# mingyuanzhou/SiD-LSG

Measured on AMD Instinct MI355X. Metric: distillation images/sec (512^2, SD1.5, kappa=1.5), higher is better.
Workload: dtype bf16

## Files before the change

### include/sidlsg_hip.h

```cpp
#ifndef SIDLSG_HIP_H
#define SIDLSG_HIP_H
#ifdef __cplusplus
extern "C" {
#endif

#define SIDLSG_OUT_F32 1
#define SIDLSG_SILU 2
#define SIDLSG_ACCUM 4

int sidlsg_gemm_bf16(const void* A, int lda, const void* W, void* C, int ldc, const float* bias, const void* res, int ldres,
                     const float* rowvec, int ld_rowvec, int rows_per_batch, int M, int N, int K, float alpha, int flags,
                     void* stream);

int sidlsg_conv3x3_bf16(const void* X, int ldx, const void* W, void* Y, int ldc, const float* bias, const void* res, int ldres,
                        const float* rowvec, int ld_rowvec, int B, int H, int Wd, int Cin, int Cout, int stride, int ups,
                        float alpha, int flags, void* stream);

int sidlsg_gemm_geglu_ok(int M, int N2, int K);
int sidlsg_gemm_geglu_bf16(const void* A, int lda, const void* W, void* H, int ldh, void* Y, int ldy, const float* bias, int M, int N2,
                           int K, void* stream);

int sidlsg_gemm_geglu_bwd_ok(int M, int F, int K);
int sidlsg_gemm_geglu_bwd_bf16(const void* dOut, int lda, const void* Wt, const void* H, void* dH, int ldh, int M, int F, int K,
                               void* stream);
int sidlsg_gemm_geglu_bf16_g2(const void* A, int lda, const void* W, const void* W1, void* H, int ldh, void* Y, int ldy, const float* bias,
                              const float* bias1, int M, int N2, int K, void* stream);
int sidlsg_gemm_geglu_bwd_bf16_g2(const void* dOut, int lda, const void* Wt, const void* Wt1, const void* H, void* dH, int ldh, int M, int F,
                                  int K, void* stream);

int sidlsg_set_workspace(void* ptr, long long bytes);
int sidlsg_set_stream_workspace(void* stream, void* ptr, long long bytes);

int sidlsg_wgrad_bf16(const void* dY, int ldy, const void* A, int lda, float* dW, float* dBias, int M, int N, int K,
                      void* stream);
int sidlsg_wgrad_assign_bf16(const void* dY, int ldy, const void* A, int lda, float* dW, float* dBias, int M, int N, int K,
                             void* stream);
int sidlsg_wgrad_group_bf16(const void* jobs, int njobs, void* stream);
int sidlsg_wgrad_group160_bf16(const void* jobs, int njobs, void* stream);
int sidlsg_conv3x3_wgrad_assign_bf16(const void* dY, int ldy, const void* X, int ldx, float* dW, float* dBias, int B, int H, int Wd,
                                     int Cin, int Cout, int stride, int ups, void* stream);
int sidlsg_debug_wgrad_blocks_per_cu(int which);
int sidlsg_debug_set_p8(int mode);
int sidlsg_conv3x3_wgrad_bf16(const void* dY, int ldy, const void* X, int ldx, float* dW, float* dBias, int B, int H, int Wd,
                              int Cin, int Cout, int stride, int ups, void* stream);

int sidlsg_groupnorm_ws_floats(int B, int HW, int C, int G);
int sidlsg_groupnorm_nchunks(int B, int HW, int C, int G);
int sidlsg_groupnorm_fwd(const void* x, const float* gamma, const float* beta, void* y, float* stats, float* ws, int B,
                         int HW, int C, int G, float eps, int silu, void* stream);
int sidlsg_groupnorm_bwd(const void* x, const void* dy, const float* stats, const float* gamma, const float* beta,
                         const void* dres, void* dx, float* dgamma, float* dbeta, float* ws, int B, int HW, int C, int G,
                         int silu, void* stream);
int sidlsg_layernorm_fwd(const void* x, const float* gamma, const float* beta, void* y, float* stats, int rows, int C,
                         float eps, void* stream);
int sidlsg_layernorm_bwd_nblocks(int rows);
int sidlsg_defer_reductions(void* stream, int on);
int sidlsg_flush_reductions(void* stream);
int sidlsg_pending_reductions(void* stream);
int sidlsg_layernorm_bwd(const void* x, const void* dy, const float* stats, const float* gamma, const void* dres, void* dx,
                         float* dgamma, float* dbeta, float* ws, int rows, int C, void* stream);

int sidlsg_gemm_bf16_g2(const void* A, int lda, const void* W, const void* W1, void* C, int ldc, const float* bias, const float* bias1,
                        const void* res, int ldres, const float* rowvec, int ld_rowvec, int rows_per_batch, int M, int N, int K,
                        float alpha, int flags, void* stream);
int sidlsg_conv3x3_bf16_g2(const void* X, int ldx, const void* W, const void* W1, void* Y, int ldc, const float* bias, const float* bias1,
                           const void* res, int ldres, const float* rowvec, int ld_rowvec, int B, int H, int Wd, int Cin, int Cout,
                           int stride, int ups, float alpha, int flags, void* stream);
int sidlsg_groupnorm_fwd_g2(const void* x, const float* gamma, const float* beta, const float* gamma1, const float* beta1, void* y,
                            float* stats, float* ws, int B, int HW, int C, int G, float eps, int silu, void* stream);
int sidlsg_groupnorm_bwd_g2(const void* x, const void* dy, const float* stats, const float* gamma, const float* beta, const float* gamma1,
                            const float* beta1, const void* dres, void* dx, float* ws, int B, int HW, int C, int G, int silu,
                            void* stream);
int sidlsg_layernorm_fwd_g2(const void* x, const float* gamma, const float* beta, const float* gamma1, const float* beta1, void* y,
                            float* stats, int rows, int C, float eps, void* stream);
int sidlsg_layernorm_bwd_g2(const void* x, const void* dy, const float* stats, const float* gamma, const float* gamma1, const void* dres,
                            void* dx, int rows, int C, void* stream);

int sidlsg_trace_enable(int max_kernels);
int sidlsg_trace_pause(int paused);
int sidlsg_trace_set_stride(int family, int stride);
int sidlsg_trace_read(int family, double* out);

int sidlsg_attn_fwd(const void* Q, const void* K, const void* V, void* O, float* LSE, int B, int H, int Nq, int Nk, int D,
                    int ldq, int ldk, int ldv, int ldo, long long bsq, long long bsk, long long bsv, long long bso,
                    void* stream);
int sidlsg_attn_bwd(const void* Q, const void* K, const void* V, const void* O, const void* dO, const float* LSE, void* dQ,
                    void* dK, void* dV, float* delta, int B, int H, int Nq, int Nk, int D, int ldq, int ldk, int ldv, int ldo,
                    long long bsq, long long bsk, long long bsv, long long bso, void* stream);
int sidlsg_attn_fwd_ps(const void* Q, const void* K, const void* V, void* O, float* LSE, int B, int H, int Nq, int Nk, int D,
                       int ldq, int ldk, int ldv, int ldo, long long bsq, long long bsk, long long bsv, long long bso,
                       void* stream);
int sidlsg_attn_bwd_ps(const void* Q, const void* K, const void* V, const void* O, const void* dO, const float* LSE, void* dQ,
                       void* dK, void* dV, float* delta, int B, int H, int Nq, int Nk, int D, int ldq, int ldk, int ldv, int ldo,
                       long long bsq, long long bsk, long long bsv, long long bso, void* stream);

int sidlsg_noisy_input(const float* x0, const float* noise, const float* s0, const float* s1, void* out, float* xt, int B,
                       int C, int HW, int Cp, int dup, void* stream);
int sidlsg_noisy_input_bwd(const void* g, const float* s0, float* dx0, int B, int C, int HW, int Cp, int dup, int accumulate,
                           void* stream);
int sidlsg_cfg_x0(const float* eps, const float* xt, const float* s0, const float* s1, float* out, int B, int C, int HW,
                  int Ce, int dup, float kappa, int predict_x0, void* stream);
int sidlsg_cfg_x0_bwd(const float* g, const float* s0, const float* s1, void* deps, float* dxt, int B, int C, int HW, int Cp,
                      int dup, float kappa, int predict_x0, void* stream);

int sidlsg_g_loss(const float* x, const float* yr, const float* yf, float* dx, float* dyr, float* dyf, float* loss, float* ws,
                  int S, int n, float alpha, float scale, void* stream);
int sidlsg_fake_loss(const float* e, const float* noise, float* de, float* loss, float* ws, int S, int n, float scale,
                     void* stream);

int sidlsg_adam_ema(float* p, float* g, float* m, float* v, float* ema, void* w_bf16, const float* hyper, long long n,
                    int zero_grad, void* stream);

int sidlsg_timestep_embed(const long long* t, void* out, int B, int dim, void* stream);
int sidlsg_silu_fwd(const void* x, void* y, long long n, void* stream);
int sidlsg_silu_bwd(const void* x, const void* dy, void* dx, long long n, void* stream);
int sidlsg_geglu_fwd(const void* h, void* y, long long M, int F, void* stream);
int sidlsg_geglu_bwd(const void* h, const void* dy, void* dh, long long M, int F, void* stream);
int sidlsg_concat2(void* a, void* b, void* out, long long M, int C1, int C2, int to_parts, void* stream);
int sidlsg_sumpool2x2(const void* g, void* out, int B, int H, int W, int C, void* stream);
int sidlsg_zero_insert2(const void* g, void* out, int B, int Ho, int Wo, int H, int W, int C, void* stream);
int sidlsg_add_bf16(const void* a, const void* b, void* o, long long n, void* stream);
int sidlsg_colsum_nchunks(int B, int rows_per_batch);
int sidlsg_colsum(const void* g, int ldg, float* per_batch, float* total, float* ws, int B, int rows_per_batch, int N,
                  void* stream);
int sidlsg_colsum_strided(const void* g, int ldg, float* per_batch, int ld_pb, float* total, int B, int rows_per_batch, int N, void* stream);
int sidlsg_cast_f32_bf16(const float* x, void* y, long long n, void* stream);
int sidlsg_cast_bf16_f32(const void* x, float* y, long long n, void* stream);
int sidlsg_transpose_w(const float* src, void* dst, int N, int K, int T, void* stream);
int sidlsg_transpose_w_batched(const void* jobs, int njobs, int nblocks, void* stream);
int sidlsg_transpose_w16_batched(const void* jobs, int njobs, int nblocks, void* stream);
int sidlsg_scale_cast_ranges(const void* jobs, int njobs, int nblocks, void* stream);

int sidlsg_bias_act(const void* x, const void* b, const void* dy, void* out, long long n, int stepB, int sizeB, int act,
                    float alpha, float gain, float clamp, int grad, int dtype, void* stream);

int sidlsg_quantize_fp8_rows(const void* src_bf16, void* dst_fp8, float* scale, int rows, int cols, void* stream);
int sidlsg_gemm_fp8w(const void* A, int lda, const void* W8, const float* wscale, void* C, int ldc, const float* bias, const void* res,
                     int ldres, const float* rowvec, int ld_rowvec, int rows_per_batch, int M, int N, int K, float alpha,
                     int flags, void* stream);
int sidlsg_conv3x3_fp8w(const void* X, int ldx, const void* W8, const float* wscale, void* Y, int ldc, const float* bias,
                        const void* res, int ldres, const float* rowvec, int ld_rowvec, int B, int H, int Wd, int Cin, int Cout,
                        int stride, int ups, float alpha, int flags, void* stream);
int sidlsg_cast_fp8(const void* src_bf16, void* dst_fp8, long long n, void* stream);
int sidlsg_conv3x3_mx8(const void* X8, int ldx, const void* W8, const float* wscale, void* Y, int ldc, const float* bias, const void* res,
                       int ldres, const float* rowvec, int ld_rowvec, int B, int H, int Wd, int Cin, int Cout, float alpha, int flags,
                       void* stream);
int sidlsg_layernorm_fwd_fp8(const void* x, const float* gamma, const float* beta, void* y8, float* stats, int rows, int C,
                             float eps, void* stream);
int sidlsg_groupnorm_fwd_fp8(const void* x, const float* gamma, const float* beta, void* y8, float* stats, float* ws, int B,
                             int HW, int C, int G, float eps, int silu, void* stream);
int sidlsg_gemm_mx8(const void* A8, int lda, const void* W8, const float* wscale, void* C, int ldc, const float* bias, const void* res,
                    int ldres, const float* rowvec, int ld_rowvec, int rows_per_batch, int M, int N, int K, float alpha,
                    int flags, void* stream);

int sidlsg_gemm_f32(const void* A, int lda, const void* W, void* C, int ldc, const float* bias, const void* res, int ldres,
                    const float* rowvec, int ld_rowvec, int rows_per_batch, int M, int N, int K, float alpha, int flags,
                    void* stream);
int sidlsg_conv3x3_f32(const void* X, int ldx, const void* W, void* Y, int ldc, const float* bias, const void* res, int ldres,
                       const float* rowvec, int ld_rowvec, int B, int H, int Wd, int Cin, int Cout, int stride, int ups,
                       float alpha, int flags, void* stream);
int sidlsg_wgrad_f32(const void* dY, int ldy, const void* A, int lda, float* dW, float* dBias, int M, int N, int K,
                     void* stream);
int sidlsg_conv3x3_wgrad_f32(const void* dY, int ldy, const void* X, int ldx, float* dW, float* dBias, int B, int H, int Wd,
                             int Cin, int Cout, int stride, int ups, void* stream);
int sidlsg_groupnorm_fwd_f32(const void* x, const float* gamma, const float* beta, void* y, float* stats, float* ws, int B,
                             int HW, int C, int G, float eps, int silu, void* stream);
int sidlsg_groupnorm_bwd_f32(const void* x, const void* dy, const float* stats, const float* gamma, const float* beta,
                             const void* dres, void* dx, float* dgamma, float* dbeta, float* ws, int B, int HW, int C, int G,
                             int silu, void* stream);
int sidlsg_layernorm_fwd_f32(const void* x, const float* gamma, const float* beta, void* y, float* stats, int rows, int C,
                             float eps, void* stream);
int sidlsg_layernorm_bwd_f32(const void* x, const void* dy, const float* stats, const float* gamma, const void* dres, void* dx,
                             float* dgamma, float* dbeta, float* ws, int rows, int C, void* stream);
int sidlsg_attn_fwd_f32(const void* Q, const void* K, const void* V, void* O, float* LSE, int B, int H, int Nq, int Nk, int D,
                        int ldq, int ldk, int ldv, int ldo, long long bsq, long long bsk, long long bsv, long long bso,
                        void* stream);
int sidlsg_attn_bwd_f32(const void* Q, const void* K, const void* V, const void* O, const void* dO, const float* LSE, void* dQ,
// ... 28 lines not shown
```

### sid_lsg_amd/csrc/attention.hip

```cpp
#include "common.h"
#include <stdlib.h>
#include <type_traits>

struct AttnParams {
    const bf16 *Q, *K, *V, *dO;
    bf16 *O, *dQ, *dK, *dV;
    float* LSE;
    const float* delta;
    float* delta_out;
    int B, H, Nq, Nk, D;
    int ldq, ldk, ldv, ldo;
    long long bsq, bsk, bsv, bso;
    float scale2;
    float scale;
    int xcd;
    int rot;
};

DEVFN void attn_block_coords(const AttnParams& p, int& bx, int& h, int& b) {
    bx = blockIdx.x; h = blockIdx.y; b = blockIdx.z;
    if (!p.xcd) return;
    const unsigned nx = gridDim.x, ny = gridDim.y, total = nx * ny * gridDim.z;
    unsigned L = blockIdx.x + nx * (blockIdx.y + ny * blockIdx.z);
    const unsigned q = total >> 3, r = total & 7, xcd = L & 7, idx = L >> 3;
// ... 532 lines not shown
        const float* dl_c = dl_s[pb_] + sub * AK_QT;
        f32x4 pp[KT][4], ds[KT][4];
        ATTN_PRIO(8, 1);
#pragma unroll
        for (int qt = 0; qt < 4; qt++) {
            Frag<DP> fq, fdo;
            frag_from_lds<DP>(fq, Qs + (qt * 16 + li) * LD, lg);
            frag_from_lds<DP>(fdo, dOs + (qt * 16 + li) * LD, lg);
#pragma unroll
            for (int kt = 0; kt < KT; kt++) {
                if constexpr (PS) {
                    const f32x4 nl = *reinterpret_cast<const f32x4*>(&lse_c[qt * 16 + lg * 4]);
                    const f32x4 nd = *reinterpret_cast<const f32x4*>(&dl_c[qt * 16 + lg * 4]);
                    const f32x4 s = mma_d<DP>(nl, fq, fk[kt]);
                    const f32x4 dp = mma_d<DP>(nd, fdo, fv[kt]);
#pragma unroll
                    for (int r = 0; r < 4; r++) {
                        const float pr = __builtin_amdgcn_exp2f(s[r]);
                        pp[kt][qt][r] = pr;
                        ds[kt][qt][r] = pr * dp[r];
                    }
                } else {
                const f32x4 s = mma_d<DP>((f32x4){0, 0, 0, 0}, fq, fk[kt]);
                const f32x4 dp = mma_d<DP>((f32x4){0, 0, 0, 0}, fdo, fv[kt]);
#pragma unroll
                for (int r = 0; r < 4; r++) {
                    const int ql = qt * 16 + lg * 4 + r;
                    const float pr = __builtin_amdgcn_exp2f(fmaf(s[r], p.scale2, -lse_c[ql]));
                    pp[kt][qt][r] = pr;
                    ds[kt][qt][r] = pr * (dp[r] - dl_c[ql]);
                }
                }
            }
        }
        ATTN_PRIO(8, 0);
        ATTN_PRIO(4, 1);
#pragma unroll
        for (int half = 0; half < 2; half++)
#pragma unroll
            for (int dt = 0; dt < DT; dt++) {
                const bf16x8 fa = tr_frag32(dOs, LD, 32 * half, dt * 16, li, lg);
                const bf16x8 fb = tr_frag32(Qs, LD, 32 * half, dt * 16, li, lg);
#pragma unroll
                for (int kt = 0; kt < KT; kt++) {
                    const bf16x8 pbv = pack_p(pp[kt][2 * half], pp[kt][2 * half + 1]);
                    const bf16x8 dsb = pack_p(ds[kt][2 * half], ds[kt][2 * half + 1]);
                    dv[kt][dt] = __builtin_amdgcn_mfma_f32_16x16x32_bf16(fa, pbv, dv[kt][dt], 0, 0, 0);
                    dk[kt][dt] = __builtin_amdgcn_mfma_f32_16x16x32_bf16(fb, dsb, dk[kt][dt], 0, 0, 0);
                }
            }
        ATTN_PRIO(4, 0);
        }
        if (more) {
            pb_ ^= 1;
            tq.commit(Qs2[pb_], LD); tdo.commit(dOs2[pb_], LD);
            if (threadIdx.x < ST) { lse_s[pb_][threadIdx.x] = lse_r; dl_s[pb_][threadIdx.x] = dl_r; }
            __syncthreads();
        }
    };
    {
        int q0 = 0;
        for (; q0 < p.Nq; q0 += ST) qtile(q0, std::true_type{});
    }
#pragma unroll
    for (int kt = 0; kt < KT; kt++) {
        if (!kok[kt]) continue;
        const int key = key0 + kt * 16 + li;
        bf16* dKp = p.dK + b * p.bsk + (long long)key * p.ldk + (long long)h * p.D;
        bf16* dVp = p.dV + b * p.bsv + (long long)key * p.ldv + (long long)h * p.D;
#pragma unroll
        for (int dt = 0; dt < DT; dt++) {
            const int d = dt * 16 + lg * 4;
            if (d + 4 <= p.D) {
                const float kf = PS ? 0.6931471805599453f : p.scale;
                bf16x4 a = {f2bf(dk[kt][dt][0] * kf), f2bf(dk[kt][dt][1] * kf), f2bf(dk[kt][dt][2] * kf), f2bf(dk[kt][dt][3] * kf)};
                bf16x4 c = {f2bf(dv[kt][dt][0]), f2bf(dv[kt][dt][1]), f2bf(dv[kt][dt][2]), f2bf(dv[kt][dt][3])};
                *reinterpret_cast<bf16x4*>(dKp + d) = a;
                *reinterpret_cast<bf16x4*>(dVp + d) = c;
            }
        }
    }
}

#define ATTN_INST(DP, PS)                                                            \
    template __global__ void attn_q_kernel<DP, 2, 0, true, PS>(AttnParams);           \
    template __global__ void attn_q_kernel<DP, 2, 0, false, PS>(AttnParams);          \
    template __global__ void attn_q_kernel<DP, 2, 1, false, PS>(AttnParams);          \
    template __global__ void attn_dkdv_kernel<DP, 1, PS>(AttnParams);
#define ATTN_INST2(DP) ATTN_INST(DP, false) ATTN_INST(DP, true)
ATTN_INST2(16) ATTN_INST2(32) ATTN_INST2(48) ATTN_INST2(64) ATTN_INST2(80) ATTN_INST2(96) ATTN_INST2(128) ATTN_INST2(160)
template __global__ void attn_dkdv_kernel<48, 2, false>(AttnParams);
template __global__ void attn_dkdv_kernel<48, 2, true>(AttnParams);
#undef ATTN_INST
#undef ATTN_INST2

template <int DP, int QT, bool PS>
static int launch_attn_q(const AttnParams& p, int mode, hipStream_t s) {
    const int qb = 4 * QT * 16;
    if (mode == 0) {
        if (p.D == DP - 8) SIDLSG_LAUNCH((attn_q_kernel<DP, QT, 0, true, PS>), dim3((p.Nq + qb - 1) / qb, p.H, p.B), dim3(256), 0, s, p);
        else SIDLSG_LAUNCH((attn_q_kernel<DP, QT, 0, false, PS>), dim3((p.Nq + qb - 1) / qb, p.H, p.B), dim3(256), 0, s, p);
    } else SIDLSG_LAUNCH((attn_q_kernel<DP, QT, 1, false, PS>), dim3((p.Nq + qb - 1) / qb, p.H, p.B), dim3(256), 0, s, p);
    return sidlsg_last_error();
}
template <int DP, int KT, bool PS>
static int launch_attn_dkdv(const AttnParams& p, hipStream_t s) {
    const int kb = 4 * KT * 16;
    SIDLSG_LAUNCH((attn_dkdv_kernel<DP, KT, PS>), dim3((p.Nk + kb - 1) / kb, p.H, p.B), dim3(256), 0, s, p);
    return sidlsg_last_error();
}
template <int DP, int QT, int KT, bool PS>
static int launch_attn(const AttnParams& p, int mode, hipStream_t s) {
    return mode == 2 ? launch_attn_dkdv<DP, KT, PS>(p, s) : launch_attn_q<DP, QT, PS>(p, mode, s);
}
static int attn_xcd_on(int mode, const AttnParams& p) {
    static const int mask = getenv("SIDLSG_ATTN_XCD") ? atoi(getenv("SIDLSG_ATTN_XCD")) : 15;
    if (!((mask >> mode) & 1)) return 0;
    return mode == 0 || (mask & 8) || (p.Nq <= 1024 && p.Nk <= 1024);
}
static int attn_rot_on(int mode, const AttnParams& p) {
    static const int mask = getenv("SIDLSG_ATTN_ROT") ? atoi(getenv("SIDLSG_ATTN_ROT")) : 6;
    return p.xcd && ((mask >> mode) & 1);
}
template <bool PS>
static int dispatch_attn(const AttnParams& p_in, int mode, hipStream_t s) {
    AttnParams p = p_in;
    p.xcd = attn_xcd_on(mode, p);
    p.rot = attn_rot_on(mode, p);
    if (p.D % 8 || p.D <= 0 || p.D > 160) return SIDLSG_EINVAL;
    const int dp = (p.D + 15) / 16 * 16;
    static const bool allow_kt2 = !(getenv("SIDLSG_ATTN_KT2") && atoi(getenv("SIDLSG_ATTN_KT2")) == 0);
    const bool kt2 = allow_kt2 && mode == 2 && p.Nk >= 1024;
    switch (dp) {
        case 16: return launch_attn<16, 2, 1, PS>(p, mode, s);
        case 32: return launch_attn<32, 2, 1, PS>(p, mode, s);
        case 48: return kt2 ? launch_attn<48, 2, 2, PS>(p, mode, s) : launch_attn<48, 2, 1, PS>(p, mode, s);
        case 64: return launch_attn<64, 2, 1, PS>(p, mode, s);
        case 80: return launch_attn<80, 2, 1, PS>(p, mode, s);
        case 96: return launch_attn<96, 2, 1, PS>(p, mode, s);
        case 128: return launch_attn<128, 2, 1, PS>(p, mode, s);
        case 160: return launch_attn<160, 2, 1, PS>(p, mode, s);
    }
    return SIDLSG_EINVAL;
}

static bool attn_spans_ok(int Nq, int Nk, int ldq, int ldk, int ldv, int ldo) {
    const long long lim = 0x7FFFFFFFLL / 2;
    return (long long)Nq * ldq < lim && (long long)Nk * ldk < lim && (long long)Nk * ldv < lim && (long long)Nq * ldo < lim;
}
static int attn_fwd_impl(bool ps, const void* Q, const void* K, const void* V, void* O, float* LSE, int B, int H, int Nq, int Nk, int D,
                         int ldq, int ldk, int ldv, int ldo, long long bsq, long long bsk, long long bsv, long long bso, void* stream) {
    if (((ldq | ldk | ldv | ldo) & 3) || !attn_spans_ok(Nq, Nk, ldq, ldk, ldv, ldo)) return SIDLSG_EINVAL;
    AttnParams p{};
    p.Q = (const bf16*)Q; p.K = (const bf16*)K; p.V = (const bf16*)V; p.O = (bf16*)O; p.LSE = LSE;
    p.B = B; p.H = H; p.Nq = Nq; p.Nk = Nk; p.D = D; p.ldq = ldq; p.ldk = ldk; p.ldv = ldv; p.ldo = ldo;
    p.bsq = bsq; p.bsk = bsk; p.bsv = bsv; p.bso = bso;
    p.scale = 1.0f / sqrtf((float)D); p.scale2 = p.scale * 1.4426950408889634f;
    return ps ? dispatch_attn<true>(p, 0, (hipStream_t)stream) : dispatch_attn<false>(p, 0, (hipStream_t)stream);
}
static int attn_bwd_impl(bool ps, const void* Q, const void* K, const void* V, const void* O, const void* dO, const float* LSE, void* dQ,
                         void* dK, void* dV, float* delta, int B, int H, int Nq, int Nk, int D, int ldq, int ldk, int ldv, int ldo,
                         long long bsq, long long bsk, long long bsv, long long bso, void* stream) {
    if (((ldq | ldk | ldv | ldo) & 3) || !attn_spans_ok(Nq, Nk, ldq, ldk, ldv, ldo)) return SIDLSG_EINVAL;
    hipStream_t s = (hipStream_t)stream;
    AttnParams p{};
    p.Q = (const bf16*)Q; p.K = (const bf16*)K; p.V = (const bf16*)V; p.dO = (const bf16*)dO;
    p.dQ = (bf16*)dQ; p.dK = (bf16*)dK; p.dV = (bf16*)dV; p.LSE = const_cast<float*>(LSE); p.delta = delta;
    p.B = B; p.H = H; p.Nq = Nq; p.Nk = Nk; p.D = D; p.ldq = ldq; p.ldk = ldk; p.ldv = ldv; p.ldo = ldo;
    p.bsq = bsq; p.bsk = bsk; p.bsv = bsv; p.bso = bso;
    p.scale = 1.0f / sqrtf((float)D); p.scale2 = p.scale * 1.4426950408889634f;
    p.O = const_cast<bf16*>((const bf16*)O); p.delta_out = delta;
    if (int e = ps ? dispatch_attn<true>(p, 1, s) : dispatch_attn<false>(p, 1, s)) return e;
    if (!dK && !dV) return SIDLSG_OK;
    if (!dK || !dV) return SIDLSG_EINVAL;
    return ps ? dispatch_attn<true>(p, 2, s) : dispatch_attn<false>(p, 2, s);
}

extern "C" {

int sidlsg_attn_fwd(const void* Q, const void* K, const void* V, void* O, float* LSE, int B, int H, int Nq, int Nk, int D,
                    int ldq, int ldk, int ldv, int ldo, long long bsq, long long bsk, long long bsv, long long bso,
                    void* stream) {
    SidlsgTraceScope ts(SIDLSG_FAM_ATTN_FWD, 4.0 * B * H * Nq * (double)Nk * D, 2.0 * B * H * D * (2.0 * Nq + 2.0 * Nk));
    return attn_fwd_impl(false, Q, K, V, O, LSE, B, H, Nq, Nk, D, ldq, ldk, ldv, ldo, bsq, bsk, bsv, bso, stream);
}

int sidlsg_attn_bwd(const void* Q, const void* K, const void* V, const void* O, const void* dO, const float* LSE, void* dQ,
                    void* dK, void* dV, float* delta, int B, int H, int Nq, int Nk, int D, int ldq, int ldk, int ldv, int ldo,
                    long long bsq, long long bsk, long long bsv, long long bso, void* stream) {
    SidlsgTraceScope ts(SIDLSG_FAM_ATTN_BWD, ((dK && dV) ? 10.0 : 6.0) * B * H * Nq * (double)Nk * D, 2.0 * B * H * D * (4.0 * Nq + ((dK && dV) ? 4.0 : 2.0) * Nk));
    return attn_bwd_impl(false, Q, K, V, O, dO, LSE, dQ, dK, dV, delta, B, H, Nq, Nk, D, ldq, ldk, ldv, ldo, bsq, bsk, bsv, bso, stream);
}

int sidlsg_attn_fwd_ps(const void* Q, const void* K, const void* V, void* O, float* LSE, int B, int H, int Nq, int Nk, int D,
                       int ldq, int ldk, int ldv, int ldo, long long bsq, long long bsk, long long bsv, long long bso,
                       void* stream) {
    SidlsgTraceScope ts(SIDLSG_FAM_ATTN_FWD, 4.0 * B * H * Nq * (double)Nk * D, 2.0 * B * H * D * (2.0 * Nq + 2.0 * Nk));
    return attn_fwd_impl(true, Q, K, V, O, LSE, B, H, Nq, Nk, D, ldq, ldk, ldv, ldo, bsq, bsk, bsv, bso, stream);
}
int sidlsg_attn_bwd_ps(const void* Q, const void* K, const void* V, const void* O, const void* dO, const float* LSE, void* dQ,
                       void* dK, void* dV, float* delta, int B, int H, int Nq, int Nk, int D, int ldq, int ldk, int ldv, int ldo,
                       long long bsq, long long bsk, long long bsv, long long bso, void* stream) {
    SidlsgTraceScope ts(SIDLSG_FAM_ATTN_BWD, ((dK && dV) ? 10.0 : 6.0) * B * H * Nq * (double)Nk * D, 2.0 * B * H * D * (4.0 * Nq + ((dK && dV) ? 4.0 : 2.0) * Nk));
    return attn_bwd_impl(true, Q, K, V, O, dO, LSE, dQ, dK, dV, delta, B, H, Nq, Nk, D, ldq, ldk, ldv, ldo, bsq, bsk, bsv, bso, stream);
}

}
```

### sid_lsg_amd/ops.py

```python
import ctypes
import weakref
import os

import torch

from ._lib import lib

BF16 = torch.bfloat16
F32 = torch.float32


def _p(t):
    return None if t is None else t.data_ptr()


def _s():
    return torch.cuda.current_stream().cuda_stream


ACT = 'act'


def _chk(t, dtype=None):
    if not t.is_cuda:
# ... 919 lines not shown
        ctx.save_for_backward(x, gamma, beta, stats, w16t)
        ctx.cfg = (B, HW, C, groups, n, res is not None)
        if fork:
            return y, x.view(x.shape)
        return y

    @staticmethod
    def backward(ctx, dy, dkeep=None):
        x, gamma, beta, stats, w16t = ctx.saved_tensors
        B, HW, C, groups, n, has_res = ctx.cfg
        if dy is None:
            return (dkeep,) + (None,) * 11
        dy = dy.contiguous()
        if dy.dtype != BF16:
            dy = dy.to(BF16)
        dn = conv3x3(dy, w16t)
        if dkeep is not None:
            dkeep = dkeep.contiguous()
            if dkeep.dtype != BF16:
                dkeep = dkeep.to(BF16)
        dx = torch.empty_like(x)
        ws = torch.empty(n, device=x.device, dtype=F32)
        lib.sidlsg_groupnorm_bwd(_p(x), _p(dn), _p(stats), _p(gamma), _p(beta), _p(dkeep) if dkeep is not None else None, _p(dx),
                                 None, None, _p(ws), B, HW, C, groups, 1, _s())
        dres = dy if (has_res and ctx.needs_input_grad[10]) else None
        return (dx,) + (None,) * 9 + (dres, None)


def _mx8_no_weight_grads(weight, gamma):
    if torch.is_grad_enabled() and ((weight is not None and weight.requires_grad) or (gamma is not None and gamma.requires_grad)):
        raise RuntimeError('the MX-fp8 path is for passes without weight gradients (frozen network, or torch.no_grad())')


def norm_conv_mx8(x, gamma, beta, eps, groups, w8, bias, w16t, weight, res=None, rowvec=None, fork=False):
    _mx8_no_weight_grads(weight, gamma)
    return _NormConvMX8.apply(x, gamma, beta, eps, groups, fork, w8, bias, w16t, weight, res, rowvec)


def norm_linear_mx8(x, gamma, beta, eps, w8, bias, w16t, weight, groups=0, silu=False, fork=False):
    _mx8_no_weight_grads(weight, gamma)
    return _NormLinearMX8.apply(x, gamma, beta, eps, groups, silu, fork, w8, bias, w16t, weight)


_ATTN_ALWAYS_KV = os.environ.get('SIDLSG_ATTN_SKIP_KV', '1') == '0'


class _Attention(torch.autograd.Function):

    @staticmethod
    def forward(ctx, qbuf, kvbuf, heads, D, qoff, koff, voff, prescaled=False):
        _chk(qbuf, ACT)
        _chk(kvbuf, qbuf.dtype)
        sfx = '_ps' if (prescaled and qbuf.dtype == BF16) else ''
        if prescaled and not sfx:
            raise RuntimeError('pre-scaled queries exist in the bf16 compute mode only')
        B, Nq, ldq = qbuf.shape
        Nk, ldk = kvbuf.shape[1], kvbuf.shape[2]
        C = heads * D
        o = torch.empty((B, Nq, C), device=qbuf.device, dtype=qbuf.dtype)
        lse = torch.empty((B, heads, Nq), device=qbuf.device, dtype=F32)
        es = qbuf.element_size()
        _fn('attn_fwd' + sfx, qbuf.dtype)(qbuf.data_ptr() + qoff * es, kvbuf.data_ptr() + koff * es, kvbuf.data_ptr() + voff * es, _p(o), _p(lse),
                                    B, heads, Nq, Nk, D, ldq, ldk, ldk, C, Nq * ldq, Nk * ldk, Nk * ldk, Nq * C, _s())
        ctx.save_for_backward(qbuf, kvbuf, o, lse)
        ctx.cfg = (heads, D, qoff, koff, voff, sfx)
        return o

    @staticmethod
    def backward(ctx, do):
        qbuf, kvbuf, o, lse = ctx.saved_tensors
        heads, D, qoff, koff, voff, sfx = ctx.cfg
        B, Nq, ldq = qbuf.shape
        Nk, ldk = kvbuf.shape[1], kvbuf.shape[2]
        C = heads * D
        do = do.contiguous()
        if do.dtype != qbuf.dtype:
            do = do.to(qbuf.dtype)
        same = qbuf.data_ptr() == kvbuf.data_ptr()
        need_kv = same or ctx.needs_input_grad[1] or _ATTN_ALWAYS_KV
        dq = torch.empty_like(qbuf)
        dkv = dq if same else (torch.empty_like(kvbuf) if need_kv else None)
        delta = torch.empty((B, heads, Nq), device=qbuf.device, dtype=F32)
        es = qbuf.element_size()
        _fn('attn_bwd' + sfx, qbuf.dtype)(qbuf.data_ptr() + qoff * es, kvbuf.data_ptr() + koff * es, kvbuf.data_ptr() + voff * es, _p(o), _p(do),
                            _p(lse), dq.data_ptr() + qoff * es, dkv.data_ptr() + koff * es if need_kv else None,
                            dkv.data_ptr() + voff * es if need_kv else None, _p(delta),
                            B, heads, Nq, Nk, D, ldq, ldk, ldk, C, Nq * ldq, Nk * ldk, Nk * ldk, Nq * C, _s())
        return dq, (None if same else dkv), None, None, None, None, None, None


def self_attention(qkv, heads, prescaled=False):
    C = qkv.shape[2] // 3
    return _Attention.apply(qkv, qkv, heads, C // heads, 0, C, 2 * C, prescaled)


def cross_attention(q, kv, heads, prescaled=False):
    C = q.shape[2]
    return _Attention.apply(q, kv, heads, C // heads, 0, 0, C, prescaled)


class _GEGLU(torch.autograd.Function):
    @staticmethod
    def forward(ctx, h):
        _chk(h, ACT)
        F2 = h.shape[-1]
        M = h.numel() // F2
        y = torch.empty(h.shape[:-1] + (F2 // 2,), device=h.device, dtype=h.dtype)
        _fn('geglu_fwd', h.dtype)(_p(h), _p(y), M, F2 // 2, _s())
        ctx.save_for_backward(h)
        return y

    @staticmethod
    def backward(ctx, dy):
        (h,) = ctx.saved_tensors
        F2 = h.shape[-1]
        dh = torch.empty_like(h)
        _fn('geglu_bwd', h.dtype)(_p(h), _p(dy.contiguous().to(h.dtype)), _p(dh), h.numel() // F2, F2 // 2, _s())
        return dh


def geglu(h):
    return _GEGLU.apply(h)


_GEGLU_FUSE_MIN_K = int(os.environ.get('SIDLSG_GEGLU_FUSE_MIN_K', '320'))


class _LinearGEGLU(torch.autograd.Function):

    @staticmethod
    def forward(ctx, x, weight, bias, w16, w16t, keep_h, with_h=False):
        _chk(x, BF16)
        M, K = x.shape
        N2 = w16.shape[0]
        y = torch.empty((M, N2 // 2), device=x.device, dtype=BF16)
        h = torch.empty((M, N2), device=x.device, dtype=BF16) if keep_h else None
        lib.sidlsg_gemm_geglu_bf16(_p(x), x.stride(0), _p(w16), _p(h), N2, _p(y), N2 // 2, _p(bias), M, N2, K, _s())
        if keep_h:
            ctx.save_for_backward(x, weight, bias, w16t, h)
        if with_h:
            ctx.set_materialize_grads(False)
            return y, h
        return y

    @staticmethod
    def backward(ctx, dy, dh=None):
        x, weight, bias, w16t, h = ctx.saved_tensors
        F2 = h.shape[-1]
        if dy is not None:
            dh_y = torch.empty_like(h)
            lib.sidlsg_geglu_bwd(_p(h), _p(dy.contiguous().to(BF16)), _p(dh_y), h.shape[0], F2 // 2, _s())
            dh = dh_y if dh is None else add(dh.contiguous().to(BF16), dh_y)
        elif dh is None:
            return None, None, None, None, None, None, None
        else:
            dh = dh.contiguous()
            if dh.dtype != BF16:
                dh = dh.to(BF16)
        dx = gemm(dh, w16t) if ctx.needs_input_grad[0] else None
        if _wants_grad(weight):
            M, K = x.shape
            need_b = _wants_grad(bias)
            assign = _take_assign(weight, BF16)
            if not _queue_dense_wgrad(dh, x, weight.grad, bias.grad if need_b else None, M, weight.shape[0], K, assign):
                wg = lib.sidlsg_wgrad_assign_bf16 if assign else lib.sidlsg_wgrad_bf16
                with _OnWgradStream(dh, x):
                    wg(_p(dh), dh.stride(0), _p(x), x.stride(0), _p(weight.grad), _p(bias.grad) if need_b else None, M, weight.shape[0], K, _s())
        elif _wants_grad(bias):
            colsum(dh, dh.shape[0], total=bias.grad)
        return dx, None, None, None, None, None, None
# ... 415 lines not shown
```

Baseline: 39.91.

## Add fused single-pass attention backward with fp32 atomic dQ workspace for D=40

```diff
diff --git a/include/sidlsg_hip.h b/include/sidlsg_hip.h
--- a/include/sidlsg_hip.h
+++ b/include/sidlsg_hip.h
@@ -93,6 +93,14 @@
 int sidlsg_attn_bwd_ps(const void* Q, const void* K, const void* V, const void* O, const void* dO, const float* LSE, void* dQ,
                        void* dK, void* dV, float* delta, int B, int H, int Nq, int Nk, int D, int ldq, int ldk, int ldv, int ldo,
                        long long bsq, long long bsk, long long bsv, long long bso, void* stream);
+int sidlsg_attn_bwd_ws(const void* Q, const void* K, const void* V, const void* O, const void* dO, const float* LSE, void* dQ,
+                       void* dK, void* dV, float* delta, float* ws, int B, int H, int Nq, int Nk, int D, int ldq, int ldk, int ldv,
+                       int ldo, long long bsq, long long bsk, long long bsv, long long bso, void* stream);
+int sidlsg_attn_bwd_ps_ws(const void* Q, const void* K, const void* V, const void* O, const void* dO, const float* LSE, void* dQ,
+                          void* dK, void* dV, float* delta, float* ws, int B, int H, int Nq, int Nk, int D, int ldq, int ldk, int ldv,
+                          int ldo, long long bsq, long long bsk, long long bsv, long long bso, void* stream);
+int sidlsg_attn_bwd_ws_floats(int B, int H, int Nq, int Nk, int D);
+int sidlsg_debug_set_attn_bwd(int mode);
 
 int sidlsg_noisy_input(const float* x0, const float* noise, const float* s0, const float* s1, void* out, float* xt, int B,
                        int C, int HW, int Cp, int dup, void* stream);
diff --git a/sid_lsg_amd/csrc/attention.hip b/sid_lsg_amd/csrc/attention.hip
--- a/sid_lsg_amd/csrc/attention.hip
+++ b/sid_lsg_amd/csrc/attention.hip
@@ -638,6 +638,250 @@
     }
 }
 
+constexpr int FB_WAVES = 8, FB_KW = 64, FB_KB = FB_WAVES * FB_KW, FB_QS = 32;
+struct AttnBwdWs { float* dq; };
+template <int DP, bool PS>
+__global__ __launch_bounds__(512, 1) void attn_bwd_fused_kernel(AttnParams p, AttnBwdWs w) {
+    constexpr int LD = tile_ld<DP>();
+    static_assert(LD == DP && DP % 16 == 0, "row image of whole 16-byte chunks, no pad columns");
+    constexpr int DT = DP / 16, KT = FB_KW / 16, QT = FB_QS / 16, C8 = DP / 8;
+    static_assert(QT == 2, "one K = 32 contraction over the slice's queries");
+    static_assert(FB_QS * C8 + 2 * FB_QS <= 256, "four staging waves");
+    constexpr int TE = lds_tile_elems<DP, FB_QS>();
+    constexpr int SLD = 48;
+    constexpr int PLD = DP - 8;
+    constexpr int NJ = (FB_QS * (DP - 8) + 255) / 256;
+    __shared__ __attribute__((aligned(16))) bf16 Qs2[2][TE];
+    __shared__ __attribute__((aligned(16))) bf16 dOs2[2][TE];
+    __shared__ __attribute__((aligned(16))) float nl_s[2][FB_QS], nd_s[2][FB_QS];
+    __shared__ __attribute__((aligned(16))) bf16 Ks[lds_tile_elems<DP, FB_KB>()];
+    __shared__ __attribute__((aligned(16))) bf16 dSs[FB_WAVES][FB_KW * SLD];
+    __shared__ __attribute__((aligned(16))) float dqp[FB_WAVES][FB_QS * PLD];
+#pragma unroll
+    for (int i = 0; i < 2; i++) { lds_tile_init<DP, FB_QS>(Qs2[i]); lds_tile_init<DP, FB_QS>(dOs2[i]); }
+    lds_tile_init<DP, FB_KB>(Ks);
+    int bx_, h_, b_;
+    attn_block_coords(p, bx_, h_, b_);
+    const int b = b_, h = h_;
+    const int lane = threadIdx.x & 63, li = lane & 15, lg = lane >> 4;
+    const int wave = __builtin_amdgcn_readfirstlane(threadIdx.x >> 6);
+    const int key0 = bx_ * FB_KB + wave * FB_KW;
+    const bf16* Kb = p.K + b * p.bsk + (long long)h * p.D;
+    const bf16* Vb = p.V + b * p.bsv + (long long)h * p.D;
+    Frag<DP> fv[KT];
+    bool kok[KT];
+#pragma unroll
+    for (int kt = 0; kt < KT; kt++) {
+        const int key = key0 + kt * 16 + li;
+        kok[kt] = key < p.Nk;
+        frag_from_global<DP>(fv[kt], Vb + (long long)(kok[kt] ? key : 0) * p.ldv, lg, p.D, kok[kt]);
+    }
+    {
+        const __amdgpu_buffer_rsrc_t rk = mk_rsrc_rows(Kb, p.Nk, p.ldk, p.D);
+#pragma unroll
+        for (int j = 0; j < FB_KB * C8 / 512; j++) {
+            const int idx = threadIdx.x + 512 * j, r = idx / C8, c = (idx - r * C8) * 8;
+            const unsigned vo = c < p.D ? (unsigned)((r * p.ldk + c) * 2) : A_OOB;
+            st8(Ks + r * LD + c, __builtin_bit_cast(bf16x8, __builtin_amdgcn_raw_buffer_load_b128(rk, vo, (unsigned)(bx_ * FB_KB) * (unsigned)p.ldk * 2u, 0)));
+        }
+    }
+    const bf16* Kw = Ks + wave * FB_KW * LD;
+    const bool kpad = key0 + FB_KW > p.Nk;
+    f32x4 dk[KT][DT], dv[KT][DT];
+#pragma unroll
+    for (int kt = 0; kt < KT; kt++)
+#pragma unroll
+        for (int i = 0; i < DT; i++) { dk[kt][i] = (f32x4){0, 0, 0, 0}; dv[kt][i] = (f32x4){0, 0, 0, 0}; }
+
+    const bool stager = wave < 4;
+    const int lt = threadIdx.x, lr = lt / C8, lc = (lt - lr * C8) * 8;
+    const __amdgpu_buffer_rsrc_t rq = mk_rsrc_rows(p.Q + b * p.bsq + (long long)h * p.D, p.Nq, p.ldq, p.D);
+    const __amdgpu_buffer_rsrc_t rdo = mk_rsrc_rows(p.dO + b * p.bso + (long long)h * p.D, p.Nq, p.ldo, p.D);
+    const unsigned voq = (lt < FB_QS * C8 && lc < p.D) ? (unsigned)((lr * p.ldq + lc) * 2) : A_OOB;
+    const unsigned vod = (lt < FB_QS * C8 && lc < p.D) ? (unsigned)((lr * p.ldo + lc) * 2) : A_OOB;
+    const float* LSEb = p.LSE + ((long long)b * p.H + h) * p.Nq;
+    const float* DLb = p.delta + ((long long)b * p.H + h) * p.Nq;
+    bf16x8 sq = zero8(), sdo = zero8();
+    float sc = 0.f;
+    bool sok = false;
+    auto stage = [&](int q0) {
+        sq = __builtin_bit_cast(bf16x8, __builtin_amdgcn_raw_buffer_load_b128(rq, voq, (unsigned)q0 * (unsigned)p.ldq * 2u, 0));
+        sdo = __builtin_bit_cast(bf16x8, __builtin_amdgcn_raw_buffer_load_b128(rdo, vod, (unsigned)q0 * (unsigned)p.ldo * 2u, 0));
+        const int j = lt - FB_QS * C8, q = q0 + (j < FB_QS ? j : j - FB_QS);
+        sok = j >= 0 && q < p.Nq;
+        if (sok) sc = j < FB_QS ? LSEb[q] : DLb[q];
+    };
+    auto commit = [&](int buf) {
+        const int j = lt - FB_QS * C8;
+        if (j < 0) { st8(Qs2[buf] + lr * LD + lc, sq); st8(dOs2[buf] + lr * LD + lc, sdo); }
+        else if (j < FB_QS) nl_s[buf][j] = sok ? -sc : -INFINITY;
+        else nd_s[buf][j - FB_QS] = sok ? -sc : 0.f;
+    };
+    const int at = threadIdx.x - 256;
+    float* wsb = w.dq + ((long long)b * p.H + h) * p.Nq * p.D;
+
+    const int nsl = (p.Nq + FB_QS - 1) / FB_QS;
+    const bool rotate = p.rot && p.Nq % FB_QS == 0 && nsl >= 2;
+    const int qbase = rotate ? (int)(((long long)bx_ * nsl) / gridDim.x) * FB_QS : 0;
+    if (stager) { stage(qbase); commit(0); }
+    __syncthreads();
+    for (int it = 0; it < nsl; it++) {
+        const int cur = it & 1;
+        int q0 = qbase + it * FB_QS;
+        if (q0 >= p.Nq) q0 -= p.Nq;
+        const bool more = it + 1 < nsl;
+        if (stager && more) stage(q0 + FB_QS >= p.Nq ? q0 + FB_QS - p.Nq : q0 + FB_QS);
+        const bf16* Qs = Qs2[cur];
+        const bf16* dOs = dOs2[cur];
+        bf16x4 pb[KT][QT], db[KT][QT];
+        ATTN_PRIO(8, 1);
+#pragma unroll
+        for (int qt = 0; qt < QT; qt++) {
+            Frag<DP> fq, fdo;
+            frag_from_lds<DP>(fq, Qs + (qt * 16 + li) * LD, lg);
+            frag_from_lds<DP>(fdo, dOs + (qt * 16 + li) * LD, lg);
+            const f32x4 nl = *reinterpret_cast<const f32x4*>(&nl_s[cur][qt * 16 + lg * 4]);
+            const f32x4 nd = *reinterpret_cast<const f32x4*>(&nd_s[cur][qt * 16 + lg * 4]);
+#pragma unroll
+            for (int kt = 0; kt < KT; kt++) {
+                Frag<DP> fk;
+                frag_from_lds<DP>(fk, Kw + (kt * 16 + li) * LD, lg);
+                if (Frag<DP>::N32 * 32 > DP && lg * 8 + (Frag<DP>::N32 - 1) * 32 >= DP) fk.w[Frag<DP>::N32 - 1] = zero8();
+                const f32x4 s = mma_d<DP>(PS ? nl : (f32x4){0, 0, 0, 0}, fq, fk);
+                const f32x4 dp = mma_d<DP>(nd, fdo, fv[kt]);
+#pragma unroll
+                for (int r = 0; r < 4; r++) {
+                    const float pr = __builtin_amdgcn_exp2f(PS ? s[r] : fmaf(s[r], p.scale2, nl[r]));
+                    pb[kt][qt][r] = f2bf(pr);
+                    db[kt][qt][r] = f2bf(pr * dp[r]);
+                }
+            }
+        }
+        ATTN_PRIO(8, 0);
+        if (kpad) {
+#pragma unroll
+            for (int kt = 0; kt < KT; kt++)
+#pragma unroll
+                for (int qt = 0; qt < QT; qt++)
+                    if (!kok[kt]) db[kt][qt] = (bf16x4){f2bf(0.f), f2bf(0.f), f2bf(0.f), f2bf(0.f)};
+        }
+        bf16* dSw = dSs[wave];
+#pragma unroll
+        for (int kt = 0; kt < KT; kt++)
+#pragma unroll
+            for (int qt = 0; qt < QT; qt++) *reinterpret_cast<bf16x4*>(dSw + (kt * 16 + li) * SLD + qt * 16 + lg * 4) = db[kt][qt];
+        ATTN_PRIO(4, 1);
+#pragma unroll
+        for (int dt = 0; dt < DT; dt++) {
+            const bf16x8 fa = tr_frag32(dOs, LD, 0, dt * 16, li, lg);
+            const bf16x8 fb = tr_frag32(Qs, LD, 0, dt * 16, li, lg);
+#pragma unroll
+            for (int kt = 0; kt < KT; kt++) {
+                const bf16x8 pbv = __builtin_shufflevector(pb[kt][0], pb[kt][1], 0, 1, 2, 3, 4, 5, 6, 7);
+                const bf16x8 dsb = __builtin_shufflevector(db[kt][0], db[kt][1], 0, 1, 2, 3, 4, 5, 6, 7);
+                dv[kt][dt] = __builtin_amdgcn_mfma_f32_16x16x32_bf16(fa, pbv, dv[kt][dt], 0, 0, 0);
+                dk[kt][dt] = __builtin_amdgcn_mfma_f32_16x16x32_bf16(fb, dsb, dk[kt][dt], 0, 0, 0);
+            }
+        }
+        f32x4 dq[DT][QT];
+#pragma unroll
+        for (int qt = 0; qt < QT; qt++) {
+#pragma unroll
+            for (int dt = 0; dt < DT; dt++) dq[dt][qt] = (f32x4){0, 0, 0, 0};
+#pragma unroll
+            for (int kb = 0; kb < 2; kb++) {
+                const bf16x8 fs = tr_frag32(dSw, SLD, kb * 32, qt * 16, li, lg);
+#pragma unroll
+                for (int dt = 0; dt < DT; dt++)
+                    dq[dt][qt] = __builtin_amdgcn_mfma_f32_16x16x32_bf16(tr_frag32(Kw, LD, kb * 32, dt * 16, li, lg), fs, dq[dt][qt], 0, 0, 0);
+            }
+        }
+        ATTN_PRIO(4, 0);
+        __syncthreads();
+        float* part = dqp[wave];
+#pragma unroll
+        for (int dt = 0; dt < DT; dt++)
+#pragma unroll
+            for (int qt = 0; qt < QT; qt++) {
+                const int d = dt * 16 + lg * 4;
+                if (d + 4 <= p.D) *reinterpret_cast<f32x4*>(part + (qt * 16 + li) * PLD + d) = dq[dt][qt];
+            }
+        if (stager && more) commit(cur ^ 1);
+        __syncthreads();
+        if (!stager) {
+            const float* pp = dqp[0];
+            const int lim = min(FB_QS, p.Nq - q0) * p.D;
+#pragma unroll
+            for (int j = 0; j < NJ; j++) {
+                const int e = at + 256 * j;
+                if (e < lim) {
+                    float t = 0.f;
+#pragma unroll
+                    for (int v = 0; v < FB_WAVES; v++) t += pp[v * FB_QS * PLD + e];
+                    unsafeAtomicAdd(wsb + (long long)q0 * p.D + e, t);
+                }
+            }
+        }
+    }
+#pragma unroll
+    for (int kt = 0; kt < KT; kt++) {
+        if (!kok[kt]) continue;
+        const int key = key0 + kt * 16 + li;
+        bf16* dKp = p.dK + b * p.bsk + (long long)key * p.ldk + (long long)h * p.D;
+        bf16* dVp = p.dV + b * p.bsv + (long long)key * p.ldv + (long long)h * p.D;
+#pragma unroll
+        for (int dt = 0; dt < DT; dt++) {
+            const int d = dt * 16 + lg * 4;
+            if (d + 4 <= p.D) {
+                const float kf = PS ? 0.6931471805599453f : p.scale;
+                bf16x4 a = {f2bf(dk[kt][dt][0] * kf), f2bf(dk[kt][dt][1] * kf), f2bf(dk[kt][dt][2] * kf), f2bf(dk[kt][dt][3] * kf)};
+                bf16x4 c = {f2bf(dv[kt][dt][0]), f2bf(dv[kt][dt][1]), f2bf(dv[kt][dt][2]), f2bf(dv[kt][dt][3])};
+                *reinterpret_cast<bf16x4*>(dKp + d) = a;
+                *reinterpret_cast<bf16x4*>(dVp + d) = c;
+            }
+        }
+    }
+}
+
+__global__ __launch_bounds__(256) void attn_bwd_prep_kernel(AttnParams p, AttnBwdWs w) {
+    const long long rows = (long long)p.B * p.Nq * p.H;
+    const long long i = blockIdx.x * 256LL + threadIdx.x;
+    if (i < rows) {
+        const int h = (int)(i % p.H);
+        const long long t = i / p.H;
+        const int q = (int)(t % p.Nq), b = (int)(t / p.Nq);
+        const bf16* o = p.O + b * p.bso + (long long)q * p.ldo + (long long)h * p.D;
+        const bf16* g = p.dO + b * p.bso + (long long)q * p.ldo + (long long)h * p.D;
+        float s = 0.f;
+        for (int c = 0; c < p.D; c += 8) {
+            const bf16x8 x = ld8(o + c), y = ld8(g + c);
+#pragma unroll
+            for (int e = 0; e < 8; e++) s += bf2f(x[e]) * bf2f(y[e]);
+        }
+        p.delta_out[((long long)b * p.H + h) * p.Nq + q] = s;
+    }
+    f32x4* z = reinterpret_cast<f32x4*>(w.dq);
+    const long long n4 = rows * p.D / 4;
+    for (long long k = i; k < n4; k += gridDim.x * 256LL) z[k] = (f32x4){0, 0, 0, 0};
+}
+
+__global__ __launch_bounds__(256) void attn_bwd_finish_kernel(AttnParams p, AttnBwdWs w) {
+    const int C8 = p.D / 8;
+    const long long n = (long long)p.B * p.Nq * p.H * C8;
+    const long long i = blockIdx.x * 256LL + threadIdx.x;
+    if (i >= n) return;
+    const int c = (int)(i % C8);
+    long long t = i / C8;
+    const int h = (int)(t % p.H);
+    t /= p.H;
+    const int q = (int)(t % p.Nq), b = (int)(t / p.Nq);
+    const float* src = w.dq + (((long long)b * p.H + h) * p.Nq + q) * p.D + c * 8;
+    const f32x4 x = *reinterpret_cast<const f32x4*>(src), y = *reinterpret_cast<const f32x4*>(src + 4);
+    bf16x8 o = {f2bf(x[0] * p.scale), f2bf(x[1] * p.scale), f2bf(x[2] * p.scale), f2bf(x[3] * p.scale),
+                f2bf(y[0] * p.scale), f2bf(y[1] * p.scale), f2bf(y[2] * p.scale), f2bf(y[3] * p.scale)};
+    st8(p.dQ + b * p.bsq + (long long)q * p.ldq + (long long)h * p.D + c * 8, o);
+}
+
 #define ATTN_INST(DP, PS)                                                            \
     template __global__ void attn_q_kernel<DP, 2, 0, true, PS>(AttnParams);           \
     template __global__ void attn_q_kernel<DP, 2, 0, false, PS>(AttnParams);          \
@@ -647,6 +891,8 @@
 ATTN_INST2(16) ATTN_INST2(32) ATTN_INST2(48) ATTN_INST2(64) ATTN_INST2(80) ATTN_INST2(96) ATTN_INST2(128) ATTN_INST2(160)
 template __global__ void attn_dkdv_kernel<48, 2, false>(AttnParams);
 template __global__ void attn_dkdv_kernel<48, 2, true>(AttnParams);
+template __global__ void attn_bwd_fused_kernel<48, false>(AttnParams, AttnBwdWs);
+template __global__ void attn_bwd_fused_kernel<48, true>(AttnParams, AttnBwdWs);
 #undef ATTN_INST
 #undef ATTN_INST2
 
@@ -714,8 +960,31 @@
     p.scale = 1.0f / sqrtf((float)D); p.scale2 = p.scale * 1.4426950408889634f;
     return ps ? dispatch_attn<true>(p, 0, (hipStream_t)stream) : dispatch_attn<false>(p, 0, (hipStream_t)stream);
 }
+static int g_attn_bwd_mode = -2;
+static int attn_bwd_mode() {
+    if (g_attn_bwd_mode == -2) g_attn_bwd_mode = getenv("SIDLSG_ATTN_FUSED_BWD") ? atoi(getenv("SIDLSG_ATTN_FUSED_BWD")) : -1;
+    return g_attn_bwd_mode;
+}
+static bool attn_bwd_fused_on(int B, int H, int Nq, int Nk, int D) {
+    const int m = attn_bwd_mode();
+    if (m == 0 || B <= 0 || H <= 0 || Nq <= 0 || Nk <= 0 || D != 40) return false;
+    return m == 1 || (Nq >= 1024 && Nk >= 1024);
+}
+static int launch_attn_bwd_fused(bool ps, const AttnParams& p_in, float* ws, hipStream_t s) {
+    AttnParams p = p_in;
+    p.xcd = attn_xcd_on(2, p);
+    p.rot = attn_rot_on(2, p);
+    const AttnBwdWs w{ws};
+    const long long rows = (long long)p.B * p.Nq * p.H;
+    SIDLSG_LAUNCH(attn_bwd_prep_kernel, dim3((unsigned)((rows + 255) / 256)), dim3(256), 0, s, p, w);
+    const dim3 grid((p.Nk + FB_KB - 1) / FB_KB, p.H, p.B);
+    if (ps) SIDLSG_LAUNCH((attn_bwd_fused_kernel<48, true>), grid, dim3(512), 0, s, p, w);
+    else SIDLSG_LAUNCH((attn_bwd_fused_kernel<48, false>), grid, dim3(512), 0, s, p, w);
+    SIDLSG_LAUNCH(attn_bwd_finish_kernel, dim3((unsigned)((rows * (p.D / 8) + 255) / 256)), dim3(256), 0, s, p, w);
+    return sidlsg_last_error();
+}
 static int attn_bwd_impl(bool ps, const void* Q, const void* K, const void* V, const void* O, const void* dO, const float* LSE, void* dQ,
-                         void* dK, void* dV, float* delta, int B, int H, int Nq, int Nk, int D, int ldq, int ldk, int ldv, int ldo,
+                         void* dK, void* dV, float* delta, float* ws, int B, int H, int Nq, int Nk, int D, int ldq, int ldk, int ldv, int ldo,
                          long long bsq, long long bsk, long long bsv, long long bso, void* stream) {
     if (((ldq | ldk | ldv | ldo) & 3) || !attn_spans_ok(Nq, Nk, ldq, ldk, ldv, ldo)) return SIDLSG_EINVAL;
     hipStream_t s = (hipStream_t)stream;
@@ -726,6 +995,7 @@
     p.bsq = bsq; p.bsk = bsk; p.bsv = bsv; p.bso = bso;
     p.scale = 1.0f / sqrtf((float)D); p.scale2 = p.scale * 1.4426950408889634f;
     p.O = const_cast<bf16*>((const bf16*)O); p.delta_out = delta;
+    if (ws && dK && dV && attn_bwd_fused_on(B, H, Nq, Nk, D)) return launch_attn_bwd_fused(ps, p, ws, s);
     if (int e = ps ? dispatch_attn<true>(p, 1, s) : dispatch_attn<false>(p, 1, s)) return e;
     if (!dK && !dV) return SIDLSG_OK;
     if (!dK || !dV) return SIDLSG_EINVAL;
@@ -745,7 +1015,7 @@
                     void* dK, void* dV, float* delta, int B, int H, int Nq, int Nk, int D, int ldq, int ldk, int ldv, int ldo,
                     long long bsq, long long bsk, long long bsv, long long bso, void* stream) {
     SidlsgTraceScope ts(SIDLSG_FAM_ATTN_BWD, ((dK && dV) ? 10.0 : 6.0) * B * H * Nq * (double)Nk * D, 2.0 * B * H * D * (4.0 * Nq + ((dK && dV) ? 4.0 : 2.0) * Nk));
-    return attn_bwd_impl(false, Q, K, V, O, dO, LSE, dQ, dK, dV, delta, B, H, Nq, Nk, D, ldq, ldk, ldv, ldo, bsq, bsk, bsv, bso, stream);
+    return attn_bwd_impl(false, Q, K, V, O, dO, LSE, dQ, dK, dV, delta, nullptr, B, H, Nq, Nk, D, ldq, ldk, ldv, ldo, bsq, bsk, bsv, bso, stream);
 }
 
 int sidlsg_attn_fwd_ps(const void* Q, const void* K, const void* V, void* O, float* LSE, int B, int H, int Nq, int Nk, int D,
@@ -758,7 +1028,31 @@
                        void* dK, void* dV, float* delta, int B, int H, int Nq, int Nk, int D, int ldq, int ldk, int ldv, int ldo,
                        long long bsq, long long bsk, long long bsv, long long bso, void* stream) {
     SidlsgTraceScope ts(SIDLSG_FAM_ATTN_BWD, ((dK && dV) ? 10.0 : 6.0) * B * H * Nq * (double)Nk * D, 2.0 * B * H * D * (4.0 * Nq + ((dK && dV) ? 4.0 : 2.0) * Nk));
-    return attn_bwd_impl(true, Q, K, V, O, dO, LSE, dQ, dK, dV, delta, B, H, Nq, Nk, D, ldq, ldk, ldv, ldo, bsq, bsk, bsv, bso, stream);
-}
-
-}
+    return attn_bwd_impl(true, Q, K, V, O, dO, LSE, dQ, dK, dV, delta, nullptr, B, H, Nq, Nk, D, ldq, ldk, ldv, ldo, bsq, bsk, bsv, bso, stream);
+}
+
+int sidlsg_attn_bwd_ws(const void* Q, const void* K, const void* V, const void* O, const void* dO, const float* LSE, void* dQ,
+                       void* dK, void* dV, float* delta, float* ws, int B, int H, int Nq, int Nk, int D, int ldq, int ldk, int ldv,
+                       int ldo, long long bsq, long long bsk, long long bsv, long long bso, void* stream) {
+    SidlsgTraceScope ts(SIDLSG_FAM_ATTN_BWD, ((dK && dV) ? 10.0 : 6.0) * B * H * Nq * (double)Nk * D, 2.0 * B * H * D * (4.0 * Nq + ((dK && dV) ? 4.0 : 2.0) * Nk));
+    return attn_bwd_impl(false, Q, K, V, O, dO, LSE, dQ, dK, dV, delta, ws, B, H, Nq, Nk, D, ldq, ldk, ldv, ldo, bsq, bsk, bsv, bso, stream);
+}
+int sidlsg_attn_bwd_ps_ws(const void* Q, const void* K, const void* V, const void* O, const void* dO, const float* LSE, void* dQ,
+                          void* dK, void* dV, float* delta, float* ws, int B, int H, int Nq, int Nk, int D, int ldq, int ldk, int ldv,
+                          int ldo, long long bsq, long long bsk, long long bsv, long long bso, void* stream) {
+    SidlsgTraceScope ts(SIDLSG_FAM_ATTN_BWD, ((dK && dV) ? 10.0 : 6.0) * B * H * Nq * (double)Nk * D, 2.0 * B * H * D * (4.0 * Nq + ((dK && dV) ? 4.0 : 2.0) * Nk));
+    return attn_bwd_impl(true, Q, K, V, O, dO, LSE, dQ, dK, dV, delta, ws, B, H, Nq, Nk, D, ldq, ldk, ldv, ldo, bsq, bsk, bsv, bso, stream);
+}
+int sidlsg_attn_bwd_ws_floats(int B, int H, int Nq, int Nk, int D) {
+    if (B <= 0 || H <= 0 || Nq <= 0 || Nk <= 0 || D <= 0 || D % 8 || D > 160) return SIDLSG_EINVAL;
+    if (!attn_bwd_fused_on(B, H, Nq, Nk, D)) return 0;
+    const long long n = (long long)B * H * Nq * D;
+    return n > 0x7FFFFFFFLL ? SIDLSG_EINVAL : (int)n;
+}
+int sidlsg_debug_set_attn_bwd(int mode) {
+    const int old = attn_bwd_mode();
+    g_attn_bwd_mode = mode;
+    return old;
+}
+
+}
diff --git a/sid_lsg_amd/ops.py b/sid_lsg_amd/ops.py
--- a/sid_lsg_amd/ops.py
+++ b/sid_lsg_amd/ops.py
@@ -1025,10 +1025,16 @@
         dkv = dq if same else (torch.empty_like(kvbuf) if need_kv else None)
         delta = torch.empty((B, heads, Nq), device=qbuf.device, dtype=F32)
         es = qbuf.element_size()
-        _fn('attn_bwd' + sfx, qbuf.dtype)(qbuf.data_ptr() + qoff * es, kvbuf.data_ptr() + koff * es, kvbuf.data_ptr() + voff * es, _p(o), _p(do),
-                            _p(lse), dq.data_ptr() + qoff * es, dkv.data_ptr() + koff * es if need_kv else None,
-                            dkv.data_ptr() + voff * es if need_kv else None, _p(delta),
-                            B, heads, Nq, Nk, D, ldq, ldk, ldk, C, Nq * ldq, Nk * ldk, Nk * ldk, Nq * C, _s())
+        args = (qbuf.data_ptr() + qoff * es, kvbuf.data_ptr() + koff * es, kvbuf.data_ptr() + voff * es, _p(o), _p(do),
+                _p(lse), dq.data_ptr() + qoff * es, dkv.data_ptr() + koff * es if need_kv else None,
+                dkv.data_ptr() + voff * es if need_kv else None, _p(delta))
+        shape = (B, heads, Nq, Nk, D, ldq, ldk, ldk, C, Nq * ldq, Nk * ldk, Nk * ldk, Nq * C, _s())
+        if qbuf.dtype == BF16:
+            n = lib.sidlsg_attn_bwd_ws_floats.raw(B, heads, Nq, Nk, D) if need_kv else 0
+            ws = torch.empty(n, device=qbuf.device, dtype=F32) if n > 0 else None
+            getattr(lib, f'sidlsg_attn_bwd{sfx}_ws')(*args, _p(ws), *shape)
+        else:
+            _fn('attn_bwd' + sfx, qbuf.dtype)(*args, *shape)
         return dq, (None if same else dkv), None, None, None, None, None, None
 
 
```

Result: no change. 40.00 (median of 6 runs) (+0.2%).
